# rhofield/rho-tts

Measured on AMD Instinct MI355X. Metric: audio-sec/wall-sec (RTF) Qwen3-TTS-1.7B batch=32, higher is better.
Workload: dtype bf16; 1 GPU; Qwen3-TTS-1.7B bf16, batch 32/GPU, 30-s reference clone, 10-word sentences (44 frames each), sampling=top-k 50 T 0.9, seeded synthetic weights; value counts delivered (post-processed) audio; global_batch=32, parallelism=dp1

## Files before the change

### rho_tts_amd/csrc/gemm.hip

```cpp
#include <hip/hip_ext.h>

#include "kernels.h"

namespace {

typedef __attribute__((ext_vector_type(8))) __bf16 bf8_t;
typedef __attribute__((ext_vector_type(8))) short s8_t;
typedef __attribute__((ext_vector_type(16))) float f16_t;
typedef __attribute__((ext_vector_type(4))) float f4_t;
typedef __attribute__((ext_vector_type(4))) int i4_t;

__device__ __forceinline__ f16_t mfma32(s8_t a, s8_t b, f16_t c) {
    return __builtin_amdgcn_mfma_f32_32x32x16_bf16(__builtin_bit_cast(bf8_t, a), __builtin_bit_cast(bf8_t, b), c, 0, 0, 0);
}

__device__ __forceinline__ unsigned pack_bf16x2(float lo, float hi) {
    return f32x2_to_bf16x2(lo, hi);
}

__global__ void k_pack_weight(const bf16_t* __restrict__ src, int N, int K, int Np, int Kp, bf16_t* __restrict__ dst) {
    const int KT = Kp / 16;
    const int64_t n_pieces = (int64_t)(Np / 32) * KT * 64;
    for (int64_t p = (int64_t)blockIdx.x * blockDim.x + threadIdx.x; p < n_pieces; p += (int64_t)gridDim.x * blockDim.x) {
        const int lane = (int)(p & 63);
// ... 345 lines not shown
    __shared__ __attribute__((aligned(16))) unsigned char lds[2 * BUF];
    const int tid = threadIdx.x, lane = tid & 63, w = tid >> 6;
    const int wm = w / WGN, wn = w % WGN;
    const int r = lane & 31, h = lane >> 5;
    int64_t rt = blockIdx.x;
    int ct = blockIdx.y;
    if (g.xcd_order) {
        const int64_t L = (int64_t)blockIdx.y * gridDim.x + blockIdx.x;
        const int xcd = (int)(L & 7);
        const int64_t j = L >> 3;
        ct = (int)(j % gridDim.y);
        rt = (j / gridDim.y) * 8 + xcd;
        if (rt * BM >= g.a.M) return;
    }
    const int64_t m0 = rt * BM;
    const int n0 = ct * BNT;
    const int kt0 = blockIdx.z * g.kt_per_split;
    int kt1 = kt0 + g.kt_per_split;
    if (kt1 > g.KT) kt1 = g.KT;
    const int n_it = (kt1 - kt0 + 1) / 2;

    int64_t row_base[2];
    int row_t[2];
    bool row_ok[2];
    int p_tap[2], p_ci[2];
#pragma unroll
    for (int i = 0; i < 2; ++i) {
        const int p = tid + i * 256;
        const int row = p >> 2, slot = p & 3;
        const int64_t m = m0 + row;
        row_ok[i] = m < g.a.M;
        int64_t b = 0, t = m;
        if (g.a.rows_out > 0) { b = m / g.a.rows_out; t = m - b * g.a.rows_out; }
        const int rows_in = g.a.rows_out > 0 ? g.a.rows_in : 0;
        row_base[i] = b * (int64_t)rows_in * g.a.Cin;
        row_t[i] = (int)t + g.a.tap_offset;
        const int kk = kt0 * 16 + slot * 8;
        p_tap[i] = kk / g.a.Cin;
        p_ci[i] = kk - p_tap[i] * g.a.Cin;
    }
    const int t_limit = g.a.rows_out > 0 ? g.a.rows_in : 0x7fffffff;

    auto load_piece = [&](int i, s8_t& dst, s8_t& dst_lo) {
        const int ti = row_t[i] + p_tap[i] * g.a.tap_stride;
        const bool ok = row_ok[i] && p_tap[i] < g.a.taps && ti >= 0 && (g.a.rows_out == 0 || ti < t_limit);
        if (ok) {
            const int64_t off = row_base[i] + (int64_t)ti * g.a.Cin + p_ci[i];
            if (A_F32) {
                const float* s = reinterpret_cast<const float*>(g.a.ptr) + off;
                const f4_t v0 = *reinterpret_cast<const f4_t*>(s), v1 = *reinterpret_cast<const f4_t*>(s + 4);
                i4_t pk;
                pk[0] = (int)pack_bf16x2(v0[0], v0[1]);
                pk[1] = (int)pack_bf16x2(v0[2], v0[3]);
                pk[2] = (int)pack_bf16x2(v1[0], v1[1]);
                pk[3] = (int)pack_bf16x2(v1[2], v1[3]);
                dst = __builtin_bit_cast(s8_t, pk);
                if (SPLIT) {
                    float rs[8];
#pragma unroll
                    for (int j = 0; j < 4; ++j) {
                        rs[j] = v0[j] - __uint_as_float(((unsigned)(unsigned short)dst[j]) << 16);
                        rs[4 + j] = v1[j] - __uint_as_float(((unsigned)(unsigned short)dst[4 + j]) << 16);
                    }
                    i4_t pl;
                    pl[0] = (int)pack_bf16x2(rs[0], rs[1]);
                    pl[1] = (int)pack_bf16x2(rs[2], rs[3]);
                    pl[2] = (int)pack_bf16x2(rs[4], rs[5]);
                    pl[3] = (int)pack_bf16x2(rs[6], rs[7]);
                    dst_lo = __builtin_bit_cast(s8_t, pl);
                }
            } else {
                dst = *reinterpret_cast<const s8_t*>(reinterpret_cast<const bf16_t*>(g.a.ptr) + off);
                if (SPLIT) dst_lo = *reinterpret_cast<const s8_t*>(reinterpret_cast<const bf16_t*>(g.a.ptr_lo) + off);
            }
        } else {
#pragma unroll
            for (int j = 0; j < 8; ++j) { dst[j] = 0; if (SPLIT) dst_lo[j] = 0; }
        }
        p_ci[i] += BK;
        while (p_ci[i] >= g.a.Cin) { p_ci[i] -= g.a.Cin; ++p_tap[i]; }
    };
    auto store_piece = [&](int i, int buf, const s8_t& v, const s8_t& v_lo) {
        const int p = tid + i * 256;
        *reinterpret_cast<s8_t*>(lds + buf * BUF + lds_a_off(p >> 2, p & 3)) = v;
        if (SPLIT) *reinterpret_cast<s8_t*>(lds + buf * BUF + BM * 64 + lds_a_off(p >> 2, p & 3)) = v_lo;
    };
    const int nt_base = (n0 >> 5) + wn * NTT;
    auto load_b = [&](int it, s8_t (&b)[NTT][2]) {
#pragma unroll
        for (int nt = 0; nt < NTT; ++nt)
#pragma unroll
            for (int kk = 0; kk < 2; ++kk) {
                const int t_n = nt_base + nt, t_k = kt0 + it * 2 + kk;
                if (t_n < g.NT && t_k < kt1)
                    b[nt][kk] = *(reinterpret_cast<const s8_t*>(g.Wp) + ((int64_t)t_n * g.KT + t_k) * 64 + lane);
                else {
#pragma unroll
                    for (int j = 0; j < 8; ++j) b[nt][kk][j] = 0;
                }
            }
    };

    f16_t acc[MT][NTT];
#pragma unroll
    for (int a = 0; a < MT; ++a)
#pragma unroll
        for (int b = 0; b < NTT; ++b)
#pragma unroll
            for (int i = 0; i < 16; ++i) acc[a][b][i] = 0.f;

    s8_t ra[2], rl[2], rb[NTT][2], rb_next[NTT][2];
    load_piece(0, ra[0], rl[0]);
    load_piece(1, ra[1], rl[1]);
    load_b(0, rb);
    store_piece(0, 0, ra[0], rl[0]);
    store_piece(1, 0, ra[1], rl[1]);
    __syncthreads();

    for (int it = 0; it < n_it; ++it) {
        const int buf = it & 1;
        const bool more = it + 1 < n_it;
        if (more) {
            load_piece(0, ra[0], rl[0]);
            load_piece(1, ra[1], rl[1]);
            load_b(it + 1, rb_next);
        }
        s8_t fa[MT][2], fl[MT][2];
#pragma unroll
        for (int mt = 0; mt < MT; ++mt)
#pragma unroll
            for (int kk = 0; kk < 2; ++kk) {
                fa[mt][kk] = *reinterpret_cast<const s8_t*>(lds + buf * BUF + lds_a_off((wm * MT + mt) * 32 + r, kk * 2 + h));
                if (SPLIT) fl[mt][kk] = *reinterpret_cast<const s8_t*>(lds + buf * BUF + BM * 64 + lds_a_off((wm * MT + mt) * 32 + r, kk * 2 + h));
            }
#pragma unroll
        for (int kk = 0; kk < 2; ++kk)
#pragma unroll
            for (int mt = 0; mt < MT; ++mt)
#pragma unroll
                for (int nt = 0; nt < NTT; ++nt) {
                    acc[mt][nt] = mfma32(fa[mt][kk], rb[nt][kk], acc[mt][nt]);
                    if (SPLIT) acc[mt][nt] = mfma32(fl[mt][kk], rb[nt][kk], acc[mt][nt]);
                }
        if (more) {
            store_piece(0, buf ^ 1, ra[0], rl[0]);
            store_piece(1, buf ^ 1, ra[1], rl[1]);
#pragma unroll
            for (int nt = 0; nt < NTT; ++nt)
#pragma unroll
                for (int kk = 0; kk < 2; ++kk) rb[nt][kk] = rb_next[nt][kk];
        }
        __syncthreads();
    }

    tile_epilogue<MT, NTT>(g, acc, m0, n0, wm, wn, r, h);
}

constexpr int MID_BK = 64;
struct MidArgs {
    const bf16_t* A;
    const bf16_t* Wp;
    float* out;
    int M, N, K, NT, KT;
    int64_t ldc;
    int seg_it;
};
template <int WM, int WN, int PF>
__global__ __launch_bounds__(256, 2) void k_gemm_mid(MidArgs g) {
    constexpr int BM = 64 * WM, BN = 64 * WN;
    constexpr int A_BYTES = BM * MID_BK * 2;
    constexpr int B_BYTES = (BN / 32) * (MID_BK / 16) * 1024;
    constexpr int NA = BM / 32, NB = BN / 32;
    __shared__ __attribute__((aligned(16))) unsigned char lds[2 * (A_BYTES + B_BYTES)];
    const int tid = threadIdx.x, lane = tid & 63, w = tid >> 6;
    const int wm = w >> 1, wn = w & 1;
    const int r = lane & 31, h = lane >> 5;
    const int n_rt = (g.M + BM - 1) / BM, n_ct = (g.N + BN - 1) / BN;
    const int xcd = blockIdx.x & 7, jj = blockIdx.x >> 3;
    const int ct = (jj / n_rt) * 8 + xcd, rt = jj % n_rt;
    if (ct >= n_ct) return;
    const int64_t m0 = (int64_t)rt * BM;
    const int n0 = ct * BN;
    const int n_it = g.K / MID_BK;
    const int a_row = tid >> 3, a_slot = tid & 7;
    const bf16_t* a_src[NA];
#pragma unroll
    for (int i = 0; i < NA; ++i) {
        int64_t m = m0 + a_row + 32 * i;
        if (m >= g.M) m = g.M - 1;
        a_src[i] = g.A + m * g.K + a_slot * 8;
    }
    const int nt0 = n0 >> 5;
    const s8_t* b_src[NB];
#pragma unroll
    for (int i = 0; i < NB; ++i) {
        const int f = (tid >> 6) + 4 * i;
        int t_n = nt0 + (f >> 2);
        if (t_n >= g.NT) t_n = g.NT - 1;
        b_src[i] = reinterpret_cast<const s8_t*>(g.Wp) + ((int64_t)t_n * g.KT + (f & 3)) * 64 + lane;
    }
    struct Regs { s8_t a[NA], b[NB]; };
    auto issue = [&](int it, Regs& rg) {
        if (it >= n_it) it = n_it - 1;
#pragma unroll
        for (int i = 0; i < NA; ++i) rg.a[i] = *reinterpret_cast<const s8_t*>(a_src[i] + (int64_t)it * MID_BK);
#pragma unroll
        for (int i = 0; i < NB; ++i) rg.b[i] = b_src[i][(int64_t)it * (MID_BK / 16) * 64];
    };
    auto stash = [&](int buf, const Regs& rg) {
        unsigned char* base = lds + buf * (A_BYTES + B_BYTES);
#pragma unroll
        for (int i = 0; i < NA; ++i) {
            const int row = a_row + 32 * i;
            *reinterpret_cast<s8_t*>(base + row * 128 + ((a_slot ^ (row & 7)) << 4)) = rg.a[i];
        }
#pragma unroll
        for (int i = 0; i < NB; ++i) *reinterpret_cast<s8_t*>(base + A_BYTES + ((tid >> 6) + 4 * i) * 1024 + lane * 16) = rg.b[i];
    };
    f16_t acc[WM][WN], tot[WM][WN];
#pragma unroll
    for (int a = 0; a < WM; ++a)
#pragma unroll
        for (int b = 0; b < WN; ++b)
#pragma unroll
            for (int i = 0; i < 16; ++i) { acc[a][b][i] = 0.f; tot[a][b][i] = 0.f; }
    int seg_left = g.seg_it;
    auto flush = [&]() {
        if (g.seg_it > 0 && --seg_left == 0) {
            seg_left = g.seg_it;
#pragma unroll
            for (int a = 0; a < WM; ++a)
#pragma unroll
                for (int b = 0; b < WN; ++b)
#pragma unroll
                    for (int i = 0; i < 16; ++i) { tot[a][b][i] += acc[a][b][i]; acc[a][b][i] = 0.f; }
        }
    };
    auto multiply = [&](int buf) {
        const unsigned char* base = lds + buf * (A_BYTES + B_BYTES);
#pragma unroll
        for (int kt = 0; kt < 4; ++kt) {
            s8_t fa[WM], fb[WN];
#pragma unroll
            for (int a = 0; a < WM; ++a) {
                const int row = (wm * WM + a) * 32 + r;
                fa[a] = *reinterpret_cast<const s8_t*>(base + row * 128 + (((kt * 2 + h) ^ (row & 7)) << 4));
            }
#pragma unroll
            for (int b = 0; b < WN; ++b) fb[b] = *reinterpret_cast<const s8_t*>(base + A_BYTES + ((wn * WN + b) * 4 + kt) * 1024 + lane * 16);
#pragma unroll
            for (int a = 0; a < WM; ++a)
#pragma unroll
                for (int b = 0; b < WN; ++b) acc[a][b] = mfma32(fa[a], fb[b], acc[a][b]);
        }
    };
    static_assert(PF % 2 == 0, "PF even");
    Regs rg[PF];
#pragma unroll
    for (int j = 0; j < PF; ++j) issue(j, rg[j]);
    stash(0, rg[0]);
    __syncthreads();
    int it = 0;
    for (; it + PF <= n_it; it += PF) {
#pragma unroll
        for (int j = 0; j < PF; ++j) {
            issue(it + j + PF, rg[j]);
            multiply(j & 1);
            flush();
            stash((j + 1) & 1, rg[(j + 1) % PF]);
            __syncthreads();
        }
    }
#pragma unroll
    for (int j = 0; j < PF - 1; ++j) {
        if (it + j < n_it) {
            multiply(j & 1);
            flush();
            stash((j + 1) & 1, rg[j + 1]);
            __syncthreads();
        }
    }
#pragma unroll
    for (int a = 0; a < WM; ++a)
#pragma unroll
        for (int b = 0; b < WN; ++b) {
            const int n = n0 + (wn * WN + b) * 32 + r;
            if (n >= g.N) continue;
#pragma unroll
            for (int i = 0; i < 16; ++i) {
                const int64_t m = m0 + (wm * WM + a) * 32 + (i & 3) + 8 * (i >> 2) + 4 * h;
                if (m < g.M) g.out[m * g.ldc + n] = g.seg_it > 0 ? tot[a][b][i] : acc[a][b][i];
            }
        }
}

template <int WGM, int WGN, int MT, int NTT, bool FUSE = false, int TAPS = 0>
__global__ __launch_bounds__(256, (WGM * MT * 32 > 128 || NTT > 3) ? 2 : 3) void k_conv_win(TiledArgs g) {
    static_assert(WGM * WGN == 4, "4 waves");
    static_assert(!FUSE || (WGN == 1 && (NTT == 3 || (NTT == 6 && MT == 1))), "the fused 1x1 conv needs every output channel of a row in one wave");
    constexpr bool WLDS = FUSE && NTT == 6;
    constexpr int BMT = WGM * MT * 32;
    constexpr int WIN_ROWS = BMT + 64;
    constexpr int NP = (WIN_ROWS * 4 + 255) / 256;
    constexpr int BNT = WGN * NTT * 32;
    constexpr int PLANE = WIN_ROWS * 64;
    constexpr int F_ROWB = 96 * 2 + 16;
// ... 275 lines not shown
    int64_t blocks = (pieces + 255) / 256;
    if (blocks > 4096) blocks = 4096;
    hipLaunchKernelGGL(k_pack_weight16, dim3((unsigned)blocks), dim3(256), 0, ctx->stream, d_src, N, K, Np, d_dst);
    RT_HIP(ctx, hipGetLastError());
    out->data16 = d_dst;
    out->Np16 = Np;
    return RT_OK;
}

int launch_pack_weight(rt_ctx* ctx, const bf16_t* d_src, int N, int K, bf16_t* d_dst, PackedW* out) {
    const int Np = (N + 31) / 32 * 32, Kp = (K + 15) / 16 * 16;
    const int64_t pieces = (int64_t)(Np / 32) * (Kp / 16) * 64;
    int64_t blocks = (pieces + 255) / 256;
    if (blocks > 4096) blocks = 4096;
    hipLaunchKernelGGL(k_pack_weight, dim3((unsigned)blocks), dim3(256), 0, ctx->stream, d_src, N, K, Np, Kp, d_dst);
    RT_HIP(ctx, hipGetLastError());
    out->data = d_dst;
    out->N = N; out->K = K; out->Np = Np; out->Kp = Kp;
    return RT_OK;
}

int skinny_pick_split(int M, int N, int K, int n_cu) {
    const int tiles = (N + 31) / 32, KT = (K + 15) / 16;
    const int target = n_cu * g_skinny_waves_per_cu;
    int s = 1;
    while (s < 32 && tiles * (s * 2) <= target && KT % (s * 2) == 0 && KT / (s * 2) >= 4 && (KT % 4 != 0 || (KT / (s * 2)) % 4 == 0)) s *= 2;
    return s;
}

int launch_gemm_skinny(rt_ctx* ctx, const bf16_t* d_a, int M, const PackedW& w, float* d_out, int64_t ldc, int split_k,
                       hipEvent_t ev_start, hipEvent_t ev_stop, int64_t slab_stride) {
    if (slab_stride <= 0) slab_stride = (int64_t)M * ldc;
    if (M < 1 || M > 64) return rt_fail(ctx, RT_ERR_INVALID, "gemm_skinny: M=%d outside 1..64", M);
    if (w.K != w.Kp) return rt_fail(ctx, RT_ERR_INVALID, "gemm_skinny: K=%d must be a multiple of 16", w.K);
    const int NT = w.Np / 32, KT = w.Kp / 16;
    if (split_k < 1 || KT % split_k) return rt_fail(ctx, RT_ERR_INVALID, "gemm_skinny: split_k=%d does not divide %d k-tiles", split_k, KT);
    dim3 grid((NT + 3) / 4, split_k);
    if (g_skinny_variant > 0 && (ev_start || ev_stop) && slab_stride == (int64_t)M * ldc) {
        const int mt = M <= 32 ? 1 : 2;
        const size_t lds = (size_t)mt * 32 * ((KT / split_k) * 32 + 16);
        if (lds <= 64 * 1024) {
            if (g_skinny_variant == 1) {
                if (mt == 1) hipExtLaunchKernelGGL((k_gemm_skinny2<1, 4>), grid, dim3(256), lds, ctx->stream, ev_start, ev_stop, 0, d_a, M, w.K, w.data, NT, KT, KT / split_k, d_out, ldc, w.N);
                else hipExtLaunchKernelGGL((k_gemm_skinny2<2, 4>), grid, dim3(256), lds, ctx->stream, ev_start, ev_stop, 0, d_a, M, w.K, w.data, NT, KT, KT / split_k, d_out, ldc, w.N);
            } else {
                if (mt == 1) hipExtLaunchKernelGGL((k_gemm_skinny2<1, 8>), grid, dim3(256), lds, ctx->stream, ev_start, ev_stop, 0, d_a, M, w.K, w.data, NT, KT, KT / split_k, d_out, ldc, w.N);
                else hipExtLaunchKernelGGL((k_gemm_skinny2<2, 8>), grid, dim3(256), lds, ctx->stream, ev_start, ev_stop, 0, d_a, M, w.K, w.data, NT, KT, KT / split_k, d_out, ldc, w.N);
            }
            RT_HIP(ctx, hipGetLastError());
            return RT_OK;
        }
    }
    if (!ev_start && !ev_stop) {
        if (M <= 32) hipLaunchKernelGGL(k_gemm_skinny<1>, grid, dim3(256), 0, ctx->stream, d_a, M, w.K, w.data, NT, KT, KT / split_k, d_out, ldc, w.N, slab_stride);
        else hipLaunchKernelGGL(k_gemm_skinny<2>, grid, dim3(256), 0, ctx->stream, d_a, M, w.K, w.data, NT, KT, KT / split_k, d_out, ldc, w.N, slab_stride);
    } else if (M <= 32)
        hipExtLaunchKernelGGL(k_gemm_skinny<1>, grid, dim3(256), 0, ctx->stream, ev_start, ev_stop, 0, d_a, M, w.K, w.data, NT, KT,
                              KT / split_k, d_out, ldc, w.N, slab_stride);
    else
        hipExtLaunchKernelGGL(k_gemm_skinny<2>, grid, dim3(256), 0, ctx->stream, ev_start, ev_stop, 0, d_a, M, w.K, w.data, NT, KT,
                              KT / split_k, d_out, ldc, w.N, slab_stride);
    RT_HIP(ctx, hipGetLastError());
    return RT_OK;
}

bool gemm_mid_shape_ok(int N, int K) { (void)N; return g_prefill_mid && K % MID_BK == 0 && K >= 128; }
bool gemm_mid_ok(int M, const PackedW& w) { return gemm_mid_shape_ok(w.N, w.K) && w.Kp == w.K && M > 64 && M <= 1024; }
int launch_gemm_mid(rt_ctx* ctx, const bf16_t* A, int M, const PackedW& w, float* out, int64_t ldc) {
    if (!gemm_mid_ok(M, w)) return rt_fail(ctx, RT_ERR_INVALID, "gemm_mid: M=%d K=%d outside its range", M, w.K);
    MidArgs g{A, w.data, out, M, w.N, w.K, w.Np / 32, w.Kp / 16, ldc, 0};
    const int S = skinny_pick_split(M, w.N, w.K, ctx->n_cu);
    if (S > 1) {
        if ((g.KT / S) % (MID_BK / 16)) return rt_fail(ctx, RT_ERR_STATE, "gemm_mid: K segments of %d k-tiles are not whole 64-deep steps (K=%d, split %d)", g.KT / S, w.K, S);
        g.seg_it = (g.KT / S) / (MID_BK / 16);
    }
    const bool big = g_prefill_mid == 1 ? (int64_t)((M + 127) / 128) * ((w.N + 63) / 64) >= 3 * ctx->n_cu : g_prefill_mid == 3;
    const int bm = big ? 128 : 64;
    const int n_rt = (M + bm - 1) / bm, n_ct = (w.N + 63) / 64;
    dim3 grid(8 * ((n_ct + 7) / 8) * n_rt);
    if (big) hipLaunchKernelGGL((k_gemm_mid<2, 1, 4>), grid, dim3(256), 0, ctx->stream, g);
    else hipLaunchKernelGGL((k_gemm_mid<1, 1, 6>), grid, dim3(256), 0, ctx->stream, g);
    RT_HIP(ctx, hipGetLastError());
    return RT_OK;
}

static bool conv_win_ok(const GemmA& a) {
    return g_conv_win && a.split && !a.is_f32 && a.ptr_lo && a.taps >= 2 && a.Cin % 32 == 0 && a.rows_out > 0 && a.rows_in == a.rows_out &&
           a.tap_offset == -(a.taps - 1) * a.tap_stride && (a.taps - 1) * a.tap_stride <= 63 && a.M % a.rows_out == 0;
}

bool conv_pair_fusable(const GemmA& a, const PackedW& w, const GemmEpi& e, const PackedW& w2) {
    const bool c96 = w.N == 96, c192 = w.N == 192 && g_fuse_conv192 && w.Np == 192 && a.taps == 7 && g_conv_unroll;
    return g_fuse_conv && g_tile96 && (c96 || c192) && w2.N == w.N && w2.K == w.N && w2.Kp == w.N && w2.Np == w.N && e.act == ACT_SNAKE && conv_win_ok(a);
}

int launch_gemm(rt_ctx* ctx, const GemmA& a, const PackedW& w, const GemmEpi& e, const PackedW* w2, const GemmEpi* e2) {
    if (a.M <= 0) return RT_OK;
    if (a.Cin % 8 || (int64_t)a.Cin * a.taps != w.K)
        return rt_fail(ctx, RT_ERR_INVALID, "gemm: A has taps=%d Cin=%d but W has K=%d", a.taps, a.Cin, w.K);
    if (e.split_k < 1 || (e.split_k > 1 && !e.out_f32)) return rt_fail(ctx, RT_ERR_INVALID, "gemm: bad split_k");
    TiledArgs g;
    g.a = a;
    g.Wp = w.data;
    g.N = w.N; g.K = w.K; g.NT = w.Np / 32; g.KT = w.Kp / 16;
    g.e = e;
    int per = (g.KT + e.split_k - 1) / e.split_k;
    per = (per + 1) / 2 * 2;
    g.kt_per_split = per;
    const bool narrow = g_tile96 && e.split_k == 1 && w.N % 96 == 0 && w.N % 128 != 0;
    const bool conv_win = conv_win_ok(a) && e.split_k == 1;
    const bool tall = conv_win && narrow && (g_conv_tall == 2 || (g_conv_tall == 1 && a.M >= 256 * 1024));
    const int bm = tall ? 256 : BM;
    const int64_t my = (a.M + bm - 1) / bm;
    if (my > 0x7fffffff) return rt_fail(ctx, RT_ERR_LENGTH, "gemm: length %lld rows too large", (long long)a.M);
    const int bn = narrow ? 96 : BN;
    const int ny = (w.N + bn - 1) / bn;
    g.xcd_order = (g_xcd_order && e.split_k == 1 && ny > 1 && my >= 64) ? 1 : 0;
    dim3 grid((unsigned)(g.xcd_order ? (my + 7) / 8 * 8 : my), ny, e.split_k);
    if (a.split && !a.is_f32 && !a.ptr_lo) return rt_fail(ctx, RT_ERR_INVALID, "gemm: split precision needs an f32 A operand or a low plane");
    if ((e.out_hi && !e.out_lo) || (e.out2_hi && (!e.out2_lo || (e.act2 != ACT_ELU && (!e.snake2_a || !e.snake2_ib)))) ||
        ((e.out_hi || e.out2_hi) && e.split_k > 1))
        return rt_fail(ctx, RT_ERR_INVALID, "gemm: incomplete hi/lo plane output");
    if (w2) {
        const bool wide = w.N == 192;
        if (!e2 || !conv_win || !narrow || (!wide && ny != 1) || (w.N != 96 && !wide) || w.Np != w.N || w2->N != w.N || w2->K != w.N || w2->Np != w.N || w2->Kp != w.N ||
            e.act != ACT_SNAKE || !e.snake_a || !e.snake_ib || e2->split_k != 1 || e2->ldc < w.N)
            return rt_fail(ctx, RT_ERR_INVALID, "gemm: this conv pair cannot be fused (96 or 192 channels, k > 1 conv with SnakeBeta, then a 1x1 conv of the same width)");
        g.Wp2 = w2->data; g.NT2 = w2->Np / 32; g.KT2 = w2->Kp / 16; g.N2 = w2->N; g.e2 = *e2;
        const bool t7f = a.taps == 7 && g_conv_unroll;
        if (wide) {
            g.xcd_order = 0;
            const dim3 grid_w((unsigned)((a.M + 127) / 128), 1, 1);
            if (!t7f) return rt_fail(ctx, RT_ERR_INVALID, "gemm: the fused 192-channel conv pair exists for k = 7 with tap unrolling only");
            hipLaunchKernelGGL((k_conv_win<4, 1, 1, 6, true, 7>), grid_w, dim3(256), 0, ctx->stream, g);
            RT_HIP(ctx, hipGetLastError());
            return RT_OK;
        }
        if (tall && t7f) hipLaunchKernelGGL((k_conv_win<4, 1, 2, 3, true, 7>), grid, dim3(256), 0, ctx->stream, g);
        else if (tall) hipLaunchKernelGGL((k_conv_win<4, 1, 2, 3, true>), grid, dim3(256), 0, ctx->stream, g);
        else hipLaunchKernelGGL((k_conv_win<4, 1, 1, 3, true>), grid, dim3(256), 0, ctx->stream, g);
        RT_HIP(ctx, hipGetLastError());
        return RT_OK;
    }
    if (conv_win) {
        const bool t7 = a.taps == 7 && g_conv_unroll;
        if (tall && t7) hipLaunchKernelGGL((k_conv_win<4, 1, 2, 3, false, 7>), grid, dim3(256), 0, ctx->stream, g);
        else if (tall) hipLaunchKernelGGL((k_conv_win<4, 1, 2, 3>), grid, dim3(256), 0, ctx->stream, g);
        else if (narrow) hipLaunchKernelGGL((k_conv_win<4, 1, 1, 3>), grid, dim3(256), 0, ctx->stream, g);
        else if (t7) hipLaunchKernelGGL((k_conv_win<2, 2, 2, 2, false, 7>), grid, dim3(256), 0, ctx->stream, g);
        else hipLaunchKernelGGL((k_conv_win<2, 2, 2, 2>), grid, dim3(256), 0, ctx->stream, g);
        RT_HIP(ctx, hipGetLastError());
        return RT_OK;
    }
#define RT_TILED(AF, SP)                                                                                          \
    do {                                                                                                          \
        if (narrow) hipLaunchKernelGGL((k_gemm_tiled<AF, SP, 4, 1, 1, 3>), grid, dim3(256), 0, ctx->stream, g);   \
        else hipLaunchKernelGGL((k_gemm_tiled<AF, SP, 2, 2, 2, 2>), grid, dim3(256), 0, ctx->stream, g);          \
    } while (0)
    if (a.split && !a.is_f32) RT_TILED(false, true);
    else if (a.split) RT_TILED(true, true);
    else if (a.is_f32) RT_TILED(true, false);
    else RT_TILED(false, false);
#undef RT_TILED
    RT_HIP(ctx, hipGetLastError());
    return RT_OK;
}
```

### rho_tts_amd/csrc/knobs.h

```cpp
#pragma once
#include "common.h"

#define RT_KNOBS(X) \
    X(0, g_skinny_variant, 0, 0, 2, "legacy skinny GEMM: 0 k_gemm_skinny, 1 k_gemm_skinny2<.,4>, 2 k_gemm_skinny2<.,8>") \
    X(100, g_decode_col, 1, 0, 1, "0 legacy 9-launch split-K decode, 1 column-owner GEMM + fused attention (5 launches per layer)") \
    X(200, g_use_graph, 1, 0, 1, "0 eager decode frames, 1 replayed from captured hipGraphs") \
    X(300, g_pred_nt, 0, 0, 1, "predictor weights: 0 cacheable loads (Infinity-Cache resident across its 15 passes), 1 non-temporal") \
    X(400, g_decode_lanes, 1, 1, 8, "decode lanes: groups of items decoding concurrently on their own streams (rt_generate)") \
    X(500, g_col_split, 0, 0, 4, "sub-tile split of narrow decode GEMMs: 0 automatic (col_split_for), 1 / 2 / 4 forced") \
    X(600, g_tile96, 1, 0, 1, "1: 128x96 workgroup tiles for N = 96 / 192 (codec decoder), 0: always 128x128") \
    X(700, g_col_rows64, 1, 0, 1, "1: one 64-row decode GEMM launch for the predictor's two-position pass, 0: two 32-row launches") \
    X(800, g_fuse_sample_embed, 1, 0, 1, "1: sampler + next-input embedding in one launch (predictor groups), 0: separate k_embed_rowsq") \
    X(900, g_prefill_fill, 3, 0, 99, "workgroups per CU a prefill GEMM's split-K aims for") \
    X(1000, g_xcd_order, 1, 0, 1, "1: tiled GEMMs run a row tile's column tiles back to back on one XCD") \
    X(1100, g_final_conv, 1, 0, 1, "the codec decoder's last conv: 1 its own LDS-window kernel, 0 a one-column GEMM") \
    X(1200, g_conv_win, 1, 0, 1, "1: k>1 convs on operand planes keep their input window in LDS (k_conv_win), 0: per-tap kernel") \
    X(1300, g_sync_parts, 0, 0, 1, "1: rt_generate waits for the stream after every frame part (bounds the dispatches in flight; profiling aid)") \
    X(1400, g_eos_check_every, 8, 1, 99, "frames between two host looks at the device-side end-of-sequence flags (1 = every frame)") \
    X(1500, g_attn_mfma, 0, 0, 2, "the talker's shared-prefix decode attention: 0 vector unit, 1 / 2 matrix cores with four rows / one row per workgroup (attention_mfma.hip); 1 measured " \
        "16.6 us per launch against 13.3 us for the vector-unit kernel at batch 32 / 460 prefix rows, so off") \
    X(1600, g_col_split4, 0, 0, 1, "1: the automatic split may go to quarter tiles (N <= 1024 on 256 CUs); measured 1.4 ms/step slower than half tiles") \
    X(1700, g_handover_every, 4, 1, 99, "queued items (n_items > rows): frames between two looks at the flags + row hand-overs.  Measured on the 1.7B model, 512 / 64 ragged texts on 32 " \
        "rows: 2 -> 487 / 445, 3 -> 489 / 445, 4 -> 491 / 447, 6 -> 485 / 445, 8 -> 477 / 428, 12 -> 475 / 434 audio-s/s (a hand-over costs ~1.4 ms, a waiting row 0.13 ms per frame)") \
    X(1800, g_conv_tall, 1, 0, 2, "k>1 convs of the 96- / 192-channel stages: 0 128-row tiles, 1 256-row tiles for long inputs, 2 always") \
    X(1900, g_prefill_mid, 1, 0, 3, "prompt prefills of 65..1024 rows: 0 split-K tiled kernel, 1 k_gemm_mid (no split-K slabs), 2 / 3 force its 64 / 128 tiles") \
    X(2000, g_col_max_rows, 64, 1, 64, "batches up to this many rows decode on the column-owner path.  Above 32 the talker's GEMMs take 64 rows per launch and the predictor's " \
        "two-position first pass runs as two 64-row launches: 715 audio-s/s at batch 64 against 510 at batch 32 (1.7B, bench.py --batch 64) - every weight byte serves twice the rows for " \
        "~1.4x the launch time") \
    X(2100, g_fuse_conv, 1, 0, 1, "1: a 96-channel k>1 conv and the 1x1 conv behind its activation run as one launch (launch_conv_pair); 0 switches the 192-channel pairs off as well") \
    X(2200, g_prefill_attn_mfma, 1, 0, 1, "prompt attention behind a shared voice prefix: 0 vector unit, 1 matrix cores") \
    X(2300, g_col_rows16, 0, 0, 1, "1: decode GEMM launches of <= 16 rows take the 128-VGPR MT = 1 instantiation (two workgroups per CU: decode lanes)") \
    X(2400, g_col_silu_x, 1, 0, 1, "1: gate/up GEMMs whose pairs are 1.5x the CUs run as one round of 1.5-pair workgroups, 0: one pair per workgroup (1.5 rounds)") \
    X(2600, g_conv_unroll, 1, 0, 1, "1: k = 7 convs run the tap-unrolled instantiation of k_conv_win, 0: the generic tap loop") \
    X(2700, g_frame_inc_fold, 0, 0, 1, "1: frame += 1 by the last workgroup of the frame's talker-input launch, 0: k_frame_inc (the fold measured 1-1.8 ms per step SLOWER)") \
    X(2800, g_pair_attn, 1, 0, 1, "1: two-position decode passes append both positions inside the fused attention launch, 0: k_qkv_post + k_attention") \
    X(2900, g_c2w_lean, 1, 0, 1, "1: rt_code2wav drops the third unit's unread residual-stream store and the waveform copy (the last conv writes the caller's buffer)") \
    X(3000, g_fuse_conv192, 1, 0, 1, "1: the 192-channel conv pairs fuse as well, weight fragments staged through LDS") \
    X(3100, g_pred_qkv_table, 1, 0, 1, "predictor passes 2..G-1: 1 layer 0's q/k/v row of the drawn code is copied from the table rt_model_finalize builds (by the launch " \
        "that embeds the code), 0 the layer-0 qkv GEMM launch runs (same bits either way)")

#define RT_KNOB_ARG(X) \
    X(0, g_skinny_waves_per_cu, 4, 1, 0x7fffffff, "legacy skinny GEMM: split-K is chosen so that about this many waves per CU stream weights")

#define RT_KNOB_EXTERN(base, name, def, lo, hi, doc) extern rt_knob name;
RT_KNOBS(RT_KNOB_EXTERN)
RT_KNOB_ARG(RT_KNOB_EXTERN)
#undef RT_KNOB_EXTERN
extern std::atomic<int> g_tune_epoch;
```

Baseline: 579.0 audio-s/s.

## Add branch-free double-stage prefetch variant of tiled GEMM K loop

Adds k_gemm_tiled_pf, a tiled GEMM whose K loop issues A loads on clamped addresses without branches, keeps two register stages of A in flight, and double-buffers B through buffer-resource loads. A FAST path steps tap and channel indices incrementally when Cin is a multiple of 32, avoiding per-iteration divisions. Dispatch routes eligible tiled GEMMs (mostly codec-decoder convs and prefill GEMMs) to the new kernel behind a default-on knob. The aim is to hide global-load latency and cut address arithmetic, at the cost of higher register pressure and lower occupancy in some instantiations.

```diff
diff --git a/rho_tts_amd/csrc/gemm.hip b/rho_tts_amd/csrc/gemm.hip
--- a/rho_tts_amd/csrc/gemm.hip
+++ b/rho_tts_amd/csrc/gemm.hip
@@ -521,6 +521,199 @@
         }
         __syncthreads();
     }
+
+    tile_epilogue<MT, NTT>(g, acc, m0, n0, wm, wn, r, h);
+}
+
+template <bool A_F32, bool SPLIT, bool FAST, int WGM, int WGN, int MT, int NTT>
+__global__ __launch_bounds__(256, (SPLIT && A_F32 && FAST && MT * NTT == 4) ? 2 : 3) void k_gemm_tiled_pf(TiledArgs g) {
+    static_assert(WGM * WGN == 4 && WGM * MT * 32 == BM, "4 waves, 128 rows");
+    constexpr int BNT = WGN * NTT * 32;
+    constexpr int PLANES = SPLIT ? 2 : 1;
+    constexpr int BUF = BM * 64 * PLANES;
+    __shared__ __attribute__((aligned(16))) unsigned char lds[2 * BUF];
+    const int tid = threadIdx.x, lane = tid & 63, w = __builtin_amdgcn_readfirstlane(tid >> 6);
+    const int wm = w / WGN, wn = w % WGN;
+    const int r = lane & 31, h = lane >> 5;
+    int64_t rt = blockIdx.x;
+    int ct = blockIdx.y;
+    if (g.xcd_order) {
+        const int64_t L = (int64_t)blockIdx.y * gridDim.x + blockIdx.x;
+        const int xcd = (int)(L & 7);
+        const int64_t j = L >> 3;
+        ct = (int)(j % gridDim.y);
+        rt = (j / gridDim.y) * 8 + xcd;
+        if (rt * BM >= g.a.M) return;
+    }
+    const int64_t m0 = rt * BM;
+    const int n0 = ct * BNT;
+    const int kt0 = blockIdx.z * g.kt_per_split;
+    int kt1 = kt0 + g.kt_per_split;
+    if (kt1 > g.KT) kt1 = g.KT;
+    const int n_it = (kt1 - kt0 + 1) / 2;
+
+    const int Cin = g.a.Cin, taps = g.a.taps, tap_stride = g.a.tap_stride;
+    const int slot = tid & 3;
+    const int t_last = g.a.rows_out > 0 ? g.a.rows_in - 1 : 0;
+    int64_t row_base[2];
+    int row_t[2];
+    bool row_ok[2];
+#pragma unroll
+    for (int i = 0; i < 2; ++i) {
+        int64_t m = m0 + (tid >> 2) + i * 64;
+        row_ok[i] = m < g.a.M;
+        if (!row_ok[i]) m = g.a.M - 1;
+        if (g.a.rows_out > 0) {
+            const int64_t b = m / g.a.rows_out;
+            row_base[i] = b * (int64_t)g.a.rows_in * Cin;
+            row_t[i] = (int)(m - b * g.a.rows_out) + g.a.tap_offset;
+        } else {
+            row_base[i] = m * Cin;
+            row_t[i] = g.a.tap_offset;
+        }
+        if (FAST) row_base[i] += slot * 8;
+    }
+    int u_tap = (kt0 * 16) / Cin, u_ci = kt0 * 16 - u_tap * Cin;
+    int k_next = kt0 * 16;
+
+    struct ARegs {
+        f4_t f[A_F32 ? 2 : 1][2];
+        s8_t s[A_F32 ? 1 : 2][PLANES];
+        bool ok[2];
+    };
+    auto issue_a = [&](ARegs& rg) {
+#pragma unroll
+        for (int i = 0; i < 2; ++i) {
+            int tap, ci;
+            if (FAST) { tap = u_tap; ci = u_ci; }
+            else { const int kk = k_next + slot * 8; tap = kk / Cin; ci = kk - tap * Cin; }
+            const int tap_c = tap < taps ? tap : taps - 1;
+            const int ti = row_t[i] + tap_c * tap_stride;
+            rg.ok[i] = row_ok[i] & (tap < taps) & (ti >= 0) & (ti <= t_last);
+            const int ti_c = ti < 0 ? 0 : (ti > t_last ? t_last : ti);
+            const int64_t off = row_base[i] + (int64_t)ti_c * Cin + ci;
+            if constexpr (A_F32) {
+                const float* s = reinterpret_cast<const float*>(g.a.ptr) + off;
+                rg.f[i][0] = *reinterpret_cast<const f4_t*>(s);
+                rg.f[i][1] = *reinterpret_cast<const f4_t*>(s + 4);
+            } else {
+                rg.s[i][0] = *reinterpret_cast<const s8_t*>(reinterpret_cast<const bf16_t*>(g.a.ptr) + off);
+                if constexpr (SPLIT) rg.s[i][PLANES - 1] = *reinterpret_cast<const s8_t*>(reinterpret_cast<const bf16_t*>(g.a.ptr_lo) + off);
+            }
+        }
+        if (FAST) {
+            u_ci += BK;
+            if (u_ci >= Cin) { u_ci = 0; ++u_tap; }
+        } else {
+            k_next += BK;
+        }
+    };
+    auto stash_a = [&](int buf, const ARegs& rg) {
+#pragma unroll
+        for (int i = 0; i < 2; ++i) {
+            i4_t hi, lo;
+            if constexpr (A_F32) {
+                const f4_t v0 = rg.f[i][0], v1 = rg.f[i][1];
+                hi[0] = (int)pack_bf16x2(v0[0], v0[1]);
+                hi[1] = (int)pack_bf16x2(v0[2], v0[3]);
+                hi[2] = (int)pack_bf16x2(v1[0], v1[1]);
+                hi[3] = (int)pack_bf16x2(v1[2], v1[3]);
+                if constexpr (SPLIT) {
+                    const s8_t d = __builtin_bit_cast(s8_t, hi);
+                    float rs[8];
+#pragma unroll
+                    for (int j = 0; j < 4; ++j) {
+                        rs[j] = v0[j] - __uint_as_float(((unsigned)(unsigned short)d[j]) << 16);
+                        rs[4 + j] = v1[j] - __uint_as_float(((unsigned)(unsigned short)d[4 + j]) << 16);
+                    }
+                    lo[0] = (int)pack_bf16x2(rs[0], rs[1]);
+                    lo[1] = (int)pack_bf16x2(rs[2], rs[3]);
+                    lo[2] = (int)pack_bf16x2(rs[4], rs[5]);
+                    lo[3] = (int)pack_bf16x2(rs[6], rs[7]);
+                }
+            } else {
+                hi = __builtin_bit_cast(i4_t, rg.s[i][0]);
+                if constexpr (SPLIT) lo = __builtin_bit_cast(i4_t, rg.s[i][PLANES - 1]);
+            }
+            const bool ok = rg.ok[i];
+            const int o = buf * BUF + lds_a_off((tid >> 2) + i * 64, slot);
+#pragma unroll
+            for (int j = 0; j < 4; ++j) hi[j] = ok ? hi[j] : 0;
+            *reinterpret_cast<i4_t*>(lds + o) = hi;
+            if constexpr (SPLIT) {
+#pragma unroll
+                for (int j = 0; j < 4; ++j) lo[j] = ok ? lo[j] : 0;
+                *reinterpret_cast<i4_t*>(lds + o + BM * 64) = lo;
+            }
+        }
+    };
+    const int nt_base = (n0 >> 5) + wn * NTT;
+    __amdgpu_buffer_rsrc_t b_rsrc[NTT];
+#pragma unroll
+    for (int nt = 0; nt < NTT; ++nt) {
+        const int t_n = nt_base + nt;
+        const bf16_t* base = g.Wp + (int64_t)(t_n < g.NT ? t_n : g.NT - 1) * g.KT * 512;
+        b_rsrc[nt] = __builtin_amdgcn_make_buffer_rsrc((void*)base, 0, t_n < g.NT ? (unsigned)kt1 * 1024u : 0u, 0x00020000);
+    }
+    auto issue_b = [&](int it, i4_t (&b)[NTT][2]) {
+        const unsigned off = (unsigned)(kt0 + it * 2) * 1024u + (unsigned)lane * 16u;
+#pragma unroll
+        for (int nt = 0; nt < NTT; ++nt)
+#pragma unroll
+            for (int kk = 0; kk < 2; ++kk)
+                b[nt][kk] = __builtin_bit_cast(i4_t, __builtin_amdgcn_raw_buffer_load_b128(b_rsrc[nt], off + kk * 1024u, 0, 0));
+    };
+
+    f16_t acc[MT][NTT];
+#pragma unroll
+    for (int a = 0; a < MT; ++a)
+#pragma unroll
+        for (int b = 0; b < NTT; ++b)
+#pragma unroll
+            for (int i = 0; i < 16; ++i) acc[a][b][i] = 0.f;
+
+    auto multiply = [&](int buf, const i4_t (&b)[NTT][2]) {
+        s8_t fa[MT][2], fl[MT][2];
+#pragma unroll
+        for (int mt = 0; mt < MT; ++mt)
+#pragma unroll
+            for (int kk = 0; kk < 2; ++kk) {
+                fa[mt][kk] = *reinterpret_cast<const s8_t*>(lds + buf * BUF + lds_a_off((wm * MT + mt) * 32 + r, kk * 2 + h));
+                if (SPLIT) fl[mt][kk] = *reinterpret_cast<const s8_t*>(lds + buf * BUF + BM * 64 + lds_a_off((wm * MT + mt) * 32 + r, kk * 2 + h));
+            }
+#pragma unroll
+        for (int kk = 0; kk < 2; ++kk)
+#pragma unroll
+            for (int mt = 0; mt < MT; ++mt)
+#pragma unroll
+                for (int nt = 0; nt < NTT; ++nt) {
+                    const s8_t fb = __builtin_bit_cast(s8_t, b[nt][kk]);
+                    acc[mt][nt] = mfma32(fa[mt][kk], fb, acc[mt][nt]);
+                    if (SPLIT) acc[mt][nt] = mfma32(fl[mt][kk], fb, acc[mt][nt]);
+                }
+    };
+
+    constexpr int PF = (SPLIT && MT * NTT == 4 && !FAST) ? 1 : 2;
+    ARegs ra[PF];
+    i4_t rb[2][NTT][2];
+    issue_a(ra[0]);
+    issue_b(0, rb[0]);
+    if constexpr (PF == 2) issue_a(ra[1]);
+    stash_a(0, ra[0]);
+    __syncthreads();
+    int it = 0;
+    for (; it + 2 <= n_it; it += 2) {
+#pragma unroll
+        for (int j = 0; j < 2; ++j) {
+            issue_b(it + j + 1, rb[(j + 1) & 1]);
+            issue_a(ra[j % PF]);
+            __builtin_amdgcn_sched_barrier(0);
+            multiply(j, rb[j]);
+            stash_a((j + 1) & 1, ra[(j + 1) % PF]);
+            __syncthreads();
+        }
+    }
+    if (it < n_it) multiply(0, rb[0]);
 
     tile_epilogue<MT, NTT>(g, acc, m0, n0, wm, wn, r, h);
 }
@@ -1102,9 +1295,19 @@
         RT_HIP(ctx, hipGetLastError());
         return RT_OK;
     }
+    const bool pf = g_tiled_loop && ((a.rows_out > 0 && a.rows_in >= 1 && a.M % a.rows_out == 0) || (a.rows_out == 0 && a.taps == 1 && a.tap_offset == 0)) &&
+                    (int64_t)g.KT * 1024 < 0x7fffffff;
+    const bool fast = a.Cin % 32 == 0;
+#define RT_TILED_PF(AF, SP, FA)                                                                                          \
+    do {                                                                                                                 \
+        if (narrow) hipLaunchKernelGGL((k_gemm_tiled_pf<AF, SP, FA, 4, 1, 1, 3>), grid, dim3(256), 0, ctx->stream, g);   \
+        else hipLaunchKernelGGL((k_gemm_tiled_pf<AF, SP, FA, 2, 2, 2, 2>), grid, dim3(256), 0, ctx->stream, g);          \
+    } while (0)
 #define RT_TILED(AF, SP)                                                                                          \
     do {                                                                                                          \
-        if (narrow) hipLaunchKernelGGL((k_gemm_tiled<AF, SP, 4, 1, 1, 3>), grid, dim3(256), 0, ctx->stream, g);   \
+        if (pf && fast) RT_TILED_PF(AF, SP, true);                                                                \
+        else if (pf) RT_TILED_PF(AF, SP, false);                                                                  \
+        else if (narrow) hipLaunchKernelGGL((k_gemm_tiled<AF, SP, 4, 1, 1, 3>), grid, dim3(256), 0, ctx->stream, g);   \
         else hipLaunchKernelGGL((k_gemm_tiled<AF, SP, 2, 2, 2, 2>), grid, dim3(256), 0, ctx->stream, g);          \
     } while (0)
     if (a.split && !a.is_f32) RT_TILED(false, true);
@@ -1112,6 +1315,7 @@
     else if (a.is_f32) RT_TILED(true, false);
     else RT_TILED(false, false);
 #undef RT_TILED
+#undef RT_TILED_PF
     RT_HIP(ctx, hipGetLastError());
     return RT_OK;
 }
diff --git a/rho_tts_amd/csrc/knobs.h b/rho_tts_amd/csrc/knobs.h
--- a/rho_tts_amd/csrc/knobs.h
+++ b/rho_tts_amd/csrc/knobs.h
@@ -37,7 +37,9 @@
     X(2900, g_c2w_lean, 1, 0, 1, "1: rt_code2wav drops the third unit's unread residual-stream store and the waveform copy (the last conv writes the caller's buffer)") \
     X(3000, g_fuse_conv192, 1, 0, 1, "1: the 192-channel conv pairs fuse as well, weight fragments staged through LDS") \
     X(3100, g_pred_qkv_table, 1, 0, 1, "predictor passes 2..G-1: 1 layer 0's q/k/v row of the drawn code is copied from the table rt_model_finalize builds (by the launch " \
-        "that embeds the code), 0 the layer-0 qkv GEMM launch runs (same bits either way)")
+        "that embeds the code), 0 the layer-0 qkv GEMM launch runs (same bits either way)") \
+    X(3200, g_tiled_loop, 1, 0, 1, "the tiled GEMM's K loop: 1 branch-free requests on clamped addresses, two register stages of A in flight (k_gemm_tiled_pf), " \
+        "0 the guarded one-stage loop (k_gemm_tiled); same bits either way")
 
 #define RT_KNOB_ARG(X) \
     X(0, g_skinny_waves_per_cu, 4, 1, 0x7fffffff, "legacy skinny GEMM: split-K is chosen so that about this many waves per CU stream weights")
```

Result: no change. 582.9 audio-s/s (median of 6 runs) (+0.7%).
